# mmottl/gpr

Hardware: AMD Instinct MI355X
Metric: FITC nLML+grad training-points/sec at n=1M m=2048 d=8 (higher is better)
Workload: dtype f64

## Files before the change

### gpr_amd/csrc/gprhip.hip

```cpp
#include <algorithm>
#include <cmath>
#include <cstring>
#include <vector>
#include <string>
#include "../../include/gprhip.h"
#include "common.h"
#include "kernels.h"
#include "mfma_gemm.h"
#include "predict_plan.h"
#include "problem_internal.h"
#include "sample_paths_host.h"

static_assert(gprhip::PLAN_TILE == gprhip::TILE, "predict_plan.h rounds to the engine's tile");

namespace gprhip {
const std::string& last_error();

__global__ __launch_bounds__(256) void normalize_kernel(double* __restrict__ x, int n, double* __restrict__ nrm) {
  __shared__ double red[256];
  double s = 0.0;
  for (int i = threadIdx.x; i < n; i += 256) s += x[i] * x[i];
  red[threadIdx.x] = s;
  __syncthreads();
  for (int o = 128; o > 0; o >>= 1) {
// ... 3736 lines not shown
  }, p);
}

int gprhip_acquire_max_value(gprhip_problem* p, const double* extremes, int n_extremes, int maximise, double var_floor,
                             const double* test_inputs, int64_t ld, int64_t nt, double* values, double* dvalues, int64_t ldg,
                             double* means, double* variances, int top_k, int64_t* top_index, double* top_values,
                             double* top_dvalues, int on_device) {
  return guarded([&] {
    auto refuse = [](const char* why) {
      set_error(std::string("gprhip_acquire_max_value: ") + why);
      throw HipFail{ST_BAD_ARG};
    };
    if (n_extremes < 1 || n_extremes > GPRHIP_MAX_EXTREMES) refuse("n_extremes must lie in 1 .. GPRHIP_MAX_EXTREMES (64)");
    if (!extremes) refuse("invalid arguments (extremes is NULL)");
    for (int j = 0; j < n_extremes; ++j)
      if (!std::isfinite(extremes[j])) refuse("the extremes must be finite");
    if (!(var_floor > 0.0) || !std::isfinite(var_floor)) refuse("var_floor must be positive and finite");
    if (top_k < 0 || top_k > GPRHIP_MAX_TOP_K) refuse("top_k must lie in 0 .. GPRHIP_MAX_TOP_K (64)");
    if (top_k > 0 && !top_index) refuse("top_k > 0 needs top_index");
    if (!values && !dvalues && !means && !variances && top_k == 0)
      refuse("nothing is requested (the four outputs are NULL and top_k is 0)");
    if (!p || !test_inputs || nt < 1) refuse("invalid arguments");
    if (p->f32) refuse("the prediction gradient is evaluated in fp64 only (GPRHIP_F32_BULK problem)");
    if (p->d > 64) refuse("at most 64 point dimensions on the kernel side (d)");
    if (on_device ? ld != p->D : ld < p->D) refuse("bad ld (need ld == D for device buffers, ld >= D for host buffers)");
    if (dvalues && (on_device ? ldg != p->D : ldg < p->D))
      refuse("bad ldg (need ldg == D for device buffers, ldg >= D for host buffers)");
    do_acquire_max_value(p, extremes, n_extremes, maximise, var_floor, test_inputs, ld, nt, values, dvalues, ldg, means, variances,
                         top_k, top_index, top_values, top_dvalues, on_device);
  }, p);
}

void check_refine_options(const char* fn, const gprhip_refine_options* opt, int64_t ns, bool any_output) {
  auto refuse = [&](const std::string& why) {
    set_error(std::string(fn) + ": " + why);
    throw HipFail{ST_BAD_ARG};
  };
  if (!opt) refuse("invalid arguments (opt is NULL)");
  if (opt->max_evals < 1 || opt->max_evals > GPRHIP_REFINE_MAX_EVALS) refuse("max_evals must lie in 1 .. GPRHIP_REFINE_MAX_EVALS (1000)");
  if (!(opt->step0 > 0.0 && opt->step0 <= 1.0)) refuse("step0 must lie in (0, 1]");
  if (!(opt->c1 >= 0.0 && opt->c1 < 1.0)) refuse("c1 must lie in [0, 1)");
  if (!(opt->shrink > 0.0 && opt->shrink < 1.0)) refuse("shrink must lie in (0, 1)");
  if (!(opt->grow >= 1.0) || !std::isfinite(opt->grow)) refuse("grow must be finite and at least 1");
  if (!(opt->xtol >= 0.0) || !std::isfinite(opt->xtol)) refuse("xtol must be finite and not negative");
  if (ns < 1 || ns > GPRHIP_REFINE_MAX_STARTS) refuse("ns must lie in 1 .. GPRHIP_REFINE_MAX_STARTS (4096)");
  if (!any_output) refuse("nothing is requested (all outputs are NULL)");
}

void check_refine_box(const char* fn, const gprhip_problem* p, const double* lower, const double* upper, const double* scale,
                      int64_t ld, const double* x_out, int64_t ldx, const double* dvalues, int64_t ldg, int on_device) {
  auto refuse = [&](const std::string& why) {
    set_error(std::string(fn) + ": " + why);
    throw HipFail{ST_BAD_ARG};
  };
  const int D = p->D;
  if (on_device ? ld != D : ld < D) refuse("bad ld (need ld == D for device buffers, ld >= D for host buffers)");
  if (x_out && (on_device ? ldx != D : ldx < D)) refuse("bad ldx (need ldx == D for device buffers, ldx >= D for host buffers)");
  if (dvalues && (on_device ? ldg != D : ldg < D)) refuse("bad ldg (need ldg == D for device buffers, ldg >= D for host buffers)");
  for (int k = 0; k < D; ++k) {
    if (!std::isfinite(lower[k]) || !std::isfinite(upper[k]) || !(lower[k] < upper[k])) refuse("lower and upper must be finite with lower < upper");
    if (scale && (!(scale[k] > 0.0) || !std::isfinite(scale[k]))) refuse("scale must be positive and finite");
  }
}

std::vector<double> refine_starts(const char* fn, gprhip_problem* p, const double* starts, int64_t ld, int64_t ns, int on_device) {
  const int D = p->D;
  std::vector<double> hs((size_t)ns * D);
  if (on_device) {
    GPR_HIP(hipSetDevice(p->device));
    GPR_HIP(hipMemcpy(hs.data(), starts, hs.size() * sizeof(double), hipMemcpyDeviceToHost));
  } else {
    for (int64_t i = 0; i < ns; ++i) std::copy(starts + i * ld, starts + i * ld + D, hs.begin() + i * D);
  }
  for (double v : hs)
    if (!std::isfinite(v)) {
      set_error(std::string(fn) + ": the starts must be finite");
      throw HipFail{ST_BAD_ARG};
    }
  return hs;
}

int gprhip_acquire_refine(gprhip_problem* p, const gprhip_acquisition* acq, const gprhip_refine_options* opt, const double* lower,
                          const double* upper, const double* scale, const double* starts, int64_t ld, int64_t ns, double* x_out,
                          int64_t ldx, double* values, double* dvalues, int64_t ldg, int* evals, int* accepted, int* status,
                          double* trace, int on_device) {
  return guarded([&] {
    const char* const fn = "gprhip_acquire_refine";
    auto refuse = [&](const std::string& why) {
      set_error(std::string(fn) + ": " + why);
      throw HipFail{ST_BAD_ARG};
    };
    check_acquisition(fn, acq);
    check_refine_options(fn, opt, ns, x_out || values || dvalues || evals || accepted || status || trace);
    if (!p || !starts || !lower || !upper) refuse("invalid arguments");
    if (p->f32) refuse("the prediction gradient is evaluated in fp64 only (GPRHIP_F32_BULK problem)");
    if (p->d > 64) refuse("at most 64 point dimensions on the kernel side (d)");
    check_refine_box(fn, p, lower, upper, scale, ld, x_out, ldx, dvalues, ldg, on_device);
    need_posterior_state(p, fn, "predict from", true, acq_wants_var(acq), true,
                         "means and their gradients are available after the next gprhip_eval");
    std::vector<double> hs = refine_starts(fn, p, starts, ld, ns, on_device);
    do_acquire_refine(p, acq, opt, lower, upper, scale, starts, hs, ns, x_out, ldx, values, dvalues, ldg, evals, accepted, status,
                      trace, on_device);
  }, p);
}

int gprhip_sample_paths_refine(gprhip_problem* p, const double* z, int64_t ldz, int nd, int maximise,
                               const gprhip_refine_options* opt, const double* lower, const double* upper, const double* scale,
                               const double* starts, int64_t ld, int64_t ns, const int* draw_of, double* x_out, int64_t ldx,
                               double* values, double* dvalues, int64_t ldg, int* evals, int* accepted, int* status,
                               double* trace, int on_device) {
  return guarded([&] {
    const char* const fn = "gprhip_sample_paths_refine";
    auto refuse = [&](const std::string& why) {
      set_error(std::string(fn) + ": " + why);
      throw HipFail{ST_BAD_ARG};
    };
    if (nd < 1 || nd > GPRHIP_MAX_DRAWS) refuse("nd must lie in 1 .. GPRHIP_MAX_DRAWS (64)");
    check_refine_options(fn, opt, ns, x_out || values || dvalues || evals || accepted || status || trace);
    if (!p || !z || !starts || !draw_of || !lower || !upper) refuse("invalid arguments");
    if (p->f32) refuse("sample paths are evaluated in fp64 only (GPRHIP_F32_BULK problem)");
    if (p->d > 64) refuse("at most 64 point dimensions on the kernel side (d)");
    if (ldz < p->m) refuse("bad ldz (need ldz >= m)");
    check_refine_box(fn, p, lower, upper, scale, ld, x_out, ldx, dvalues, ldg, on_device);
    for (int64_t i = 0; i < ns; ++i)
      if (draw_of[i] < 0 || draw_of[i] >= nd) refuse("draw_of must lie in 0 .. nd - 1");
    need_posterior_state(p, fn, "draw from", true, true, true, "draws are available after the next gprhip_eval");
    std::vector<double> hs = refine_starts(fn, p, starts, ld, ns, on_device);
    do_sample_paths_refine(p, z, ldz, nd, maximise, opt, lower, upper, scale, hs, ns, draw_of, x_out, ldx, values, dvalues, ldg,
                           evals, accepted, status, trace, on_device);
  }, p);
}

int gprhip_sample_paths(gprhip_problem* p, const double* z, int64_t ldz, int ns, const double* test_inputs, int64_t ld, int64_t nt,
                        const double* eps, int64_t lde, int predictive, double* samples, int64_t lds, int maximise, int top_k,
                        int64_t* top_index, double* top_values, double* top_dvalues, int on_device) {
  return guarded([&] {
    SpCall c;
    c.have_p = p != nullptr;
    if (p) {
      c.D = p->D; c.d = p->d; c.m = p->m; c.f32 = p->f32;
    }
    c.z = z; c.ldz = ldz; c.ns = ns; c.test_inputs = test_inputs; c.ld = ld; c.nt = nt; c.eps = eps; c.lde = lde;
    c.samples = samples; c.lds = lds; c.top_k = top_k; c.top_index = top_index; c.on_device = on_device;
    if (const char* why = sp_check_args(c)) {
      set_error(std::string("gprhip_sample_paths: ") + why);
      throw HipFail{ST_BAD_ARG};
    }
    do_sample_paths(p, z, ldz, ns, test_inputs, ld, nt, eps, lde, predictive, samples, lds, maximise, top_k, top_index,
                    top_values, top_dvalues, on_device);
  }, p);
}

int gprhip_train_stats(gprhip_problem* p, double* means, double* sums) {
  return guarded([&] {
    if (!p || !sums) {
      set_error("gprhip_train_stats: invalid arguments");
      throw HipFail{ST_BAD_ARG};
    }
    if (p->f32) do_train_stats<float>(p, means, sums);
    else do_train_stats<double>(p, means, sums);
  });
}

int gprhip_covariances(gprhip_problem* p, const double* test_inputs, int64_t ld, int64_t nt, int kind,
                       int predictive, double* cov) {
  return guarded([&] {
    if (!p || !test_inputs || !cov || nt < 1 || ld < p->D || (kind != 0 && kind != 1) || nt > (1 << 20)) {
      set_error("gprhip_covariances: invalid arguments");
      throw HipFail{ST_BAD_ARG};
    }
    do_covariances(p, test_inputs, ld, nt, kind, predictive, cov);
  });
}

int gprhip_cov_samples(gprhip_problem* p, const double* cov, int64_t ld, int64_t nt, double add_diag,
                       double jitter, const double* means, const double* z, int64_t ns, double* samples) {
  return guarded([&] {
    if (!p || !cov || !means || !z || !samples || nt < 1 || ns < 1 || ld < nt || nt > (1 << 20)) {
      set_error("gprhip_cov_samples: invalid arguments");
      throw HipFail{ST_BAD_ARG};
    }
    do_cov_samples(p, cov, ld, nt, add_diag, jitter, means, z, ns, samples);
  });
}

int gprhip_co_variance_coeffs(gprhip_problem* p, double* chol_km, double* r_mat) {
  return guarded([&] {
    if (!p) {
      set_error("gprhip_co_variance_coeffs: invalid arguments");
      throw HipFail{ST_BAD_ARG};
    }
    do_co_variance_coeffs(p, chol_km, r_mat);
  });
}

int gprhip_load_predictor(gprhip_problem* p, const gprhip_hypers* h, const double* coeffs, const double* chol_km,
                          const double* r_mat) {
  return guarded([&] {
    if (!p || !h || (chol_km == nullptr) != (r_mat == nullptr) || (!coeffs && !chol_km)) {
      set_error("gprhip_load_predictor: invalid arguments");
      throw HipFail{ST_BAD_ARG};
    }
    do_load_predictor(p, h, coeffs, chol_km, r_mat);
  });
}

int gprhip_observe(gprhip_problem* p, const double* inputs, int64_t ld, const double* targets, int k, double* dlog_evidence,
                   int on_device) {
  return guarded([&] {
    const char* why = nullptr;
    if (!p || !inputs) why = "invalid arguments (problem or inputs NULL)";
    else if (k < 1 || k > GPRHIP_MAX_OBSERVE) why = "k must lie in 1 .. GPRHIP_MAX_OBSERVE (64)";
    else if (on_device ? ld != p->D : ld < p->D) why = "bad ld (need ld == D for device buffers, ld >= D for host buffers)";
    else if (p->f32) why = "the update runs in fp64 only (GPRHIP_F32_BULK problem)";
    else if (p->d > 64) why = "at most 64 point dimensions on the kernel side (d)";
    if (why) {
      set_error(std::string("gprhip_observe: ") + why);
      throw HipFail{ST_BAD_ARG};
    }
    need_observe_state(p, "gprhip_observe");
    if ((targets == nullptr) != (p->h.model_only != 0)) {
      set_error(p->h.model_only ? "gprhip_observe: the model state has no targets (model_only, or a predictor loaded without "
                                  "coefficients): targets must be NULL"
                                : "gprhip_observe: the model state has targets: targets must not be NULL");
      throw HipFail{ST_BAD_ARG};
    }
    do_observe(p, inputs, ld, targets, k, dlog_evidence, on_device);
  }, p);
}

int gprhip_posterior_save(gprhip_problem* p) {
  return guarded([&] {
    if (!p) {
      set_error("gprhip_posterior_save: NULL problem");
      throw HipFail{ST_BAD_ARG};
    }
    do_posterior_save(p);
  });
}

int gprhip_posterior_restore(gprhip_problem* p) {
  return guarded([&] {
    if (!p) {
      set_error("gprhip_posterior_restore: NULL problem");
      throw HipFail{ST_BAD_ARG};
    }
    do_posterior_restore(p);
  });
}

int64_t gprhip_observed_count(const gprhip_problem* p) { return p ? p->n_observed : 0; }

int gprhip_condition(gprhip_problem* p, double* cond_km, double* coeff_error_bound) {
  return guarded([&] {
    if (!p) {
      set_error("gprhip_condition: NULL problem");
      throw HipFail{ST_BAD_ARG};
    }
    need_model(p, "gprhip_condition");
    const double c = condition_km(p);
    if (cond_km) *cond_km = c;
    if (coeff_error_bound) *coeff_error_bound = c * (p->f32 ? 5.9604644775390625e-8 : 1.1102230246251565e-16);
  });
}

int gprhip_sync(gprhip_problem* p) {
  return guarded([&] {
    if (!p) {
      set_error("gprhip_sync: NULL problem");
      throw HipFail{ST_BAD_ARG};
    }
    GPR_HIP(hipSetDevice(p->device));
    GPR_HIP(hipStreamSynchronize(p->stream));
  });
}

void* gprhip_stream(gprhip_problem* p) { return p ? (void*)p->stream : nullptr; }

int gprhip_set_timing(gprhip_problem* p, int level) {
  return guarded([&] {
    if (!p || level < 0 || level > 2) {
      set_error("gprhip_set_timing: invalid arguments");
      throw HipFail{ST_BAD_ARG};
    }
    p->timer.kernel = level >= 1;
    p->timer.on = level >= 2;
  });
}

int gprhip_debug_fetch(gprhip_problem* p, const char* name, double* out, int64_t len) {
  return guarded([&] {
    if (!p || !out) {
      set_error("gprhip_debug_fetch: NULL argument");
      throw HipFail{ST_BAD_ARG};
    }
    const double* src = nullptr;
    int64_t avail = 0;
    std::string nm = name ? name : "";
    if (nm == "r") { src = p->r; avail = p->n; }
    else if (nm == "is") { src = p->is; avail = p->n; }
    else if (nm == "v") { src = p->v; avail = p->n; }
    else if (nm == "w") { src = p->w; avail = p->n; }
    else if (nm == "t") { src = p->tvec; avail = p->m; }
    else if (nm == "w_mat" || nm == "x_rows") {
      need_model(p, "gprhip_debug_fetch");
      if (!p->want_grad) {
        set_error("gprhip_debug_fetch: the last evaluation was evidence-only");
        throw HipFail{ST_STATE};
      }
      GPR_HIP(hipSetDevice(p->device));
      const int m = p->m, mp = p->mp;
      if (nm == "w_mat") {
        if (len < (int64_t)m * m) {
          set_error("gprhip_debug_fetch: \"w_mat\" needs m*m doubles");
          throw HipFail{ST_BAD_ARG};
        }
        std::vector<double> h((size_t)mp * mp);
        GPR_HIP(hipMemcpyAsync(h.data(), p->wmat, h.size() * sizeof(double), hipMemcpyDeviceToHost, p->stream));
        GPR_HIP(hipStreamSynchronize(p->stream));
        for (int c = 0; c < m; ++c)
          for (int r = 0; r < m; ++r) out[(size_t)c * m + r] = h[(size_t)r * mp + c];
        return;
      }
      const int64_t rows = len / m;
      if (!p->x_last || p->f32 || rows < 1 || rows > p->rows_of(0)) {
        set_error("gprhip_debug_fetch: \"x_rows\" needs an fp64 problem whose rows fit one chunk, and len = rows*m");
        throw HipFail{ST_BAD_ARG};
      }
      std::vector<double> h((size_t)rows * mp);
      GPR_HIP(hipMemcpyAsync(h.data(), p->x_last, h.size() * sizeof(double), hipMemcpyDeviceToHost, p->stream));
      GPR_HIP(hipStreamSynchronize(p->stream));
      for (int c = 0; c < m; ++c)
        for (int64_t r = 0; r < rows; ++r) out[(size_t)c * rows + r] = h[(size_t)r * mp + c];
      return;
    }
    else if (nm == "km" || nm == "knm_rows") {
      need_model(p, "gprhip_debug_fetch");
      GPR_HIP(hipSetDevice(p->device));
      const int m = p->m, mp = p->mp;
      if (nm == "km") {
        if (len < (int64_t)m * m) {
          set_error("gprhip_debug_fetch: \"km\" needs m*m doubles");
          throw HipFail{ST_BAD_ARG};
        }
        std::vector<double> h((size_t)mp * mp);
        GPR_HIP(hipMemcpyAsync(h.data(), p->km, h.size() * sizeof(double), hipMemcpyDeviceToHost, p->stream));
        GPR_HIP(hipStreamSynchronize(p->stream));
        for (int c = 0; c < m; ++c)
          for (int r = 0; r < m; ++r) out[(size_t)c * m + r] = (r <= c) ? h[(size_t)r * mp + c] : 0.0;
        return;
      }
      const int64_t rows = len / m;
      if (rows < 1 || rows > p->rows_of(0) || !p->have_inputs) {
        set_error("gprhip_debug_fetch: \"knm_rows\" needs len = rows*m with 1 <= rows <= the first row chunk");
        throw HipFail{ST_BAD_ARG};
      }
      void* const kbuf = (p->x_last == p->bufA) ? p->bufB : p->bufA;
      std::vector<double> h((size_t)rows * mp);
      if (p->f32) {
        cov_chunk<float>(p, 0, static_cast<float*>(kbuf));
        std::vector<float> hf((size_t)rows * mp);
        GPR_HIP(hipMemcpyAsync(hf.data(), kbuf, hf.size() * sizeof(float), hipMemcpyDeviceToHost, p->stream));
        GPR_HIP(hipStreamSynchronize(p->stream));
        for (size_t i = 0; i < hf.size(); ++i) h[i] = hf[i];
      } else {
        cov_chunk<double>(p, 0, static_cast<double*>(kbuf));
        GPR_HIP(hipMemcpyAsync(h.data(), kbuf, h.size() * sizeof(double), hipMemcpyDeviceToHost, p->stream));
        GPR_HIP(hipStreamSynchronize(p->stream));
      }
      for (int c = 0; c < m; ++c)
        for (int64_t r = 0; r < rows; ++r) out[(size_t)c * rows + r] = h[(size_t)r * mp + c];
      return;
    }
    else if (nm == "uinv" || nm == "rinv") {
      need_model(p, "gprhip_debug_fetch");
      if (!p->have_factors) {
        set_error("gprhip_debug_fetch: \"" + nm + "\" needs the factors of an evaluation, or of a predictor loaded with "
                  "co-variance coefficients (chol_km, r_mat)");
        throw HipFail{ST_STATE};
      }
      if (len < (int64_t)p->m * p->m) {
        set_error("gprhip_debug_fetch: \"" + nm + "\" needs m*m doubles");
        throw HipFail{ST_BAD_ARG};
      }
      GPR_HIP(hipSetDevice(p->device));
      fetch_upper_fortran(p, nm == "uinv" ? p->uinv : p->rinv, out);
      return;
    }
    else if (nm == "rtil" || nm == "bvec") {
      need_model(p, "gprhip_debug_fetch");
      if (!p->have_factors || (nm == "bvec" && (p->h.model_only || p->multi_state))) {
        set_error("gprhip_debug_fetch: \"" + nm + "\" needs the factors of an evaluation, or of a predictor loaded with "
                  "co-variance coefficients (chol_km, r_mat)" + (nm == "bvec" ? ", and a single target vector" : ""));
        throw HipFail{ST_STATE};
      }
      if (len < (nm == "rtil" ? (int64_t)p->m * p->m : (int64_t)p->m)) {
        set_error("gprhip_debug_fetch: \"" + nm + "\" needs " + (nm == "rtil" ? "m*m" : "m") + " doubles");
        throw HipFail{ST_BAD_ARG};
      }
      GPR_HIP(hipSetDevice(p->device));
      if (nm == "rtil") {
        fetch_upper_fortran(p, p->bmat, out);
        return;
      }
      if (!p->have_b) {
        DevBuf tmp;
        ensure_b(p, tmp.get<double>(p->mp));
        GPR_HIP(hipStreamSynchronize(p->stream));
      }
      GPR_HIP(hipMemcpyAsync(out, p->bvec, (size_t)p->m * sizeof(double), hipMemcpyDeviceToHost, p->stream));
      GPR_HIP(hipStreamSynchronize(p->stream));
      return;
    }
    else if (nm == "pg_m") {
      need_model(p, "gprhip_debug_fetch");
      if (!p->pg_m || !p->pg_m_valid) {
        set_error("gprhip_debug_fetch: \"pg_m\" needs M of the current model state: it is formed by the first "
                  "gprhip_predict_input_grad or gprhip_acquire call that asks for a variance part with K and G in memory");
        throw HipFail{ST_STATE};
      }
      const int64_t m = p->m, mp = p->mp;
      if (len < m * m) {
        set_error("gprhip_debug_fetch: \"pg_m\" needs m*m doubles");
        throw HipFail{ST_BAD_ARG};
      }
      const int64_t w = len >= mp * mp ? mp : m;
      GPR_HIP(hipSetDevice(p->device));
      std::vector<double> h((size_t)mp * mp);
      GPR_HIP(hipMemcpyAsync(h.data(), p->pg_m, h.size() * sizeof(double), hipMemcpyDeviceToHost, p->stream));
      GPR_HIP(hipStreamSynchronize(p->stream));
      for (int64_t c = 0; c < w; ++c)
        for (int64_t r = 0; r < w; ++r) out[(size_t)(c * w + r)] = h[(size_t)(r * mp + c)];
      return;
    }
    else if (nm == "sp_a") {
      need_model(p, "gprhip_debug_fetch");
      if (!p->sp_coef || p->sp_ns_last < 1) {
        set_error("gprhip_debug_fetch: \"sp_a\" needs the weights of a gprhip_sample_paths or gprhip_sample_paths_refine "
                  "call on the current model state");
        throw HipFail{ST_STATE};
      }
      const int64_t m = p->m, mp = p->mp, ns = p->sp_ns_last;
      if (len < m * ns) {
        set_error("gprhip_debug_fetch: \"sp_a\" needs m doubles for each draw of that call");
        throw HipFail{ST_BAD_ARG};
      }
      const bool padded = len >= mp * SP_MAX_DRAWS;
      const int64_t rows = padded ? mp : m, cols = padded ? SP_MAX_DRAWS : ns;
      GPR_HIP(hipSetDevice(p->device));
      std::vector<double> h((size_t)mp * SP_MAX_DRAWS);
      GPR_HIP(hipMemcpyAsync(h.data(), p->sp_coef + mp * SP_MAX_DRAWS, h.size() * sizeof(double), hipMemcpyDeviceToHost, p->stream));
      GPR_HIP(hipStreamSynchronize(p->stream));
      for (int64_t c = 0; c < cols; ++c)
        for (int64_t r = 0; r < rows; ++r) out[(size_t)(c * rows + r)] = h[(size_t)(r * SP_MAX_DRAWS + c)];
      return;
    }
    else {
      set_error("gprhip_debug_fetch: unknown name");
      throw HipFail{ST_BAD_ARG};
    }
    if (len > avail) len = avail;
    GPR_HIP(hipSetDevice(p->device));
    GPR_HIP(hipStreamSynchronize(p->stream));
    if (avail == p->m || p->nchunks == 1) {
      GPR_HIP(hipMemcpy(out, src, (size_t)len * sizeof(double), hipMemcpyDeviceToHost));
    } else {
      for (int c = 0; c < p->nchunks; ++c) {
        int64_t lo = (int64_t)c * p->chunk;
        if (lo >= len) break;
        int64_t cnt = std::min<int64_t>(p->rows_of(c), len - lo);
        GPR_HIP(hipMemcpy(out + lo, src + lo, (size_t)cnt * sizeof(double), hipMemcpyDeviceToHost));
      }
    }
  });
}

int gprhip_last_timings(gprhip_problem* p, const char** names, float* ms, int cap) {
  if (!p || !names || !ms) return 0;
  int n = (int)std::min<size_t>(p->tnames.size(), (size_t)cap);
  for (int i = 0; i < n; ++i) {
    names[i] = p->tnames[i].c_str();
    ms[i] = p->tms[i];
  }
  return n;
}

}
```

### gpr_amd/csrc/grad_mfma.hip

```cpp
#include "kernels.h"
#include "exp_fast.h"

namespace gprhip {

namespace {

typedef double gd4 __attribute__((ext_vector_type(4)));
__device__ __forceinline__ gd4 mfma4(double a, double b, gd4 c) {
  return __builtin_amdgcn_mfma_f64_16x16x4f64(a, b, c, 0, 0, 0);
}
__device__ __forceinline__ double wsum(double v) {
#pragma unroll
  for (int o = 32; o > 0; o >>= 1) v += __shfl_xor(v, o);
  return v;
}

constexpr int G_RC = 64;

template <int KS4, int DT, int BT, typename TS, bool KR = false>
__global__ __launch_bounds__(256, (DT + BT <= 4 && KS4 <= 8) ? 2 : 1) void grad_mfma_kernel(GradArgs<TS> a) {
  constexpr int DP = DT * 16, LDP = DP + 1;
  constexpr int BP = BT > 0 ? BT * 16 : 1, LDB = BP + 1;
  constexpr bool PF = (DT <= 2 && BT <= 2);
  constexpr int NBUF = PF ? 2 : 1;
  __shared__ double ps[KR ? 1 : NBUF * G_RC * LDP];
  __shared__ double bs[BT > 0 ? NBUF * G_RC * LDB : 1];
  __shared__ double pn[KR ? 1 : NBUF * G_RC];
  __shared__ double red[4][2];
  __shared__ double sh[DP];
  const int tid = threadIdx.x, lane = tid & 63, wv = tid >> 6;
  if (tid < DP) sh[tid] = (a.shift && tid < a.d) ? a.shift[tid] : 0.0;
  __syncthreads();
  const int l15 = lane & 15, lq = lane >> 4;
  const int cb = blockIdx.x * 128 + wv * 32;
  const ExpK ek = exp_consts();

  double zf[2][KS4], zn[2];
  bool live_c[2];
#pragma unroll
  for (int jt = 0; jt < 2; ++jt) {
    const int col = cb + jt * 16 + l15;
    live_c[jt] = col < a.m;
    double s2 = 0.0;
    if constexpr (!KR) {
#pragma unroll
      for (int s = 0; s < KS4; ++s) {
        const int k = 4 * s + lq;
        const double z = (live_c[jt] && k < a.d) ? a.Z[(int64_t)col * a.d + k] - sh[k] : 0.0;
        zf[jt][s] = z;
        s2 += z * z;
      }
      s2 += __shfl_xor(s2, 16);
      s2 += __shfl_xor(s2, 32);
    }
    zn[jt] = s2;
  }
  gd4 g[DT][2], gb[BT > 0 ? BT : 1][2];
#pragma unroll
  for (int t = 0; t < DT; ++t)
#pragma unroll
    for (int jt = 0; jt < 2; ++jt) g[t][jt] = (gd4){0, 0, 0, 0};
#pragma unroll
  for (int t = 0; t < (BT > 0 ? BT : 1); ++t)
#pragma unroll
    for (int jt = 0; jt < 2; ++jt) gb[t][jt] = (gd4){0, 0, 0, 0};
  double cs[2] = {0.0, 0.0}, sE = 0.0, sED = 0.0;

  const int r0 = blockIdx.y * a.slab;
  const int r1 = min(a.rows, r0 + a.slab);

  auto load_x = [&](int first, double (&xv)[2][4]) {
#pragma unroll
    for (int jt = 0; jt < 2; ++jt)
#pragma unroll
      for (int r = 0; r < 4; ++r) {
        const int row = first + lq + 4 * r;
        const int64_t off = (int64_t)row * a.mp + cb + jt * 16 + l15;
        if constexpr (KR) xv[jt][r] = (row < r1) ? (double)a.X[off] * (double)a.K[off] : 0.0;
        else xv[jt][r] = (row < r1) ? (double)a.X[off] : 0.0;
      }
  };
  auto tile = [&](const double* psb, const double* bsb, const double* pnb, int rb, int rt, const double (&xv)[2][4]) {
    double ev[2][4];
#pragma unroll
    for (int jt = 0; jt < 2; ++jt) {
      if constexpr (KR) {
#pragma unroll
        for (int r = 0; r < 4; ++r) {
          const double e = live_c[jt] ? xv[jt][r] : 0.0;
          ev[jt][r] = e;
          cs[jt] += e;
          sE += e;
        }
      } else {
        gd4 s4 = (gd4){0, 0, 0, 0};
#pragma unroll
        for (int s = 0; s < KS4; ++s) s4 = mfma4(psb[(rt * 16 + l15) * LDP + 4 * s + lq], zf[jt][s], s4);
#pragma unroll
        for (int r = 0; r < 4; ++r) {
          const int lr = rt * 16 + lq + 4 * r;
          const double dist = fmax(pnb[lr] + zn[jt] - 2.0 * s4[r], 0.0);
          const double kv = exp_fast(a.log_sf2 + a.inv_ell2_05 * dist, ek);
          const double e = (live_c[jt] && rb + lr < r1) ? xv[jt][r] * kv : 0.0;
          ev[jt][r] = e;
          cs[jt] += e;
          sE += e;
          sED += e * dist;
        }
      }
    }
#pragma unroll
    for (int r = 0; r < 4; ++r) {
      const int prow = (rt * 16 + 4 * r + lq);
      if (BT == 0) {
#pragma unroll
        for (int t = 0; t < DT; ++t) {
          const double ap = psb[prow * LDP + t * 16 + l15];
          g[t][0] = mfma4(ap, ev[0][r], g[t][0]);
          g[t][1] = mfma4(ap, ev[1][r], g[t][1]);
        }
      }
      if (BT > 0) {
#pragma unroll
        for (int t = 0; t < (BT > 0 ? BT : 1); ++t) {
          const double ab = bsb[prow * LDB + t * 16 + l15];
          gb[t][0] = mfma4(ab, ev[0][r], gb[t][0]);
          gb[t][1] = mfma4(ab, ev[1][r], gb[t][1]);
        }
      }
    }
  };

  if constexpr (PF) {
    constexpr int RPP = 256 / DP, NPV = G_RC / RPP;
    constexpr int RPB = 256 / BP, NBV = BT > 0 ? G_RC / RPB : 1;
    const int sr = tid / DP, sk = tid % DP;
    const int br_ = tid / BP, bk = tid % BP;
    double pv[NPV], bv[NBV];
    auto fetch_pts = [&](int rb) {
      if constexpr (!KR) {
#pragma unroll
        for (int j = 0; j < NPV; ++j) {
          const int row = rb + sr + RPP * j;
          pv[j] = (sk < a.d && row < r1) ? a.pts[(int64_t)row * a.d + sk] - sh[sk] : 0.0;
        }
      }
      if constexpr (BT > 0) {
#pragma unroll
        for (int j = 0; j < NBV; ++j) {
          const int row = rb + br_ + RPB * j;
          bv[j] = (bk < a.D && row < r1) ? a.big[(int64_t)row * a.D + bk] : 0.0;
        }
      }
    };
    auto store_pts = [&](int buf) {
      if constexpr (!KR) {
#pragma unroll
        for (int j = 0; j < NPV; ++j) {
          const int r = sr + RPP * j;
          ps[buf * G_RC * LDP + r * LDP + sk] = pv[j];
          double s2 = pv[j] * pv[j];
          s2 += __shfl_xor(s2, 1);
          s2 += __shfl_xor(s2, 2);
          s2 += __shfl_xor(s2, 4);
          s2 += __shfl_xor(s2, 8);
          if constexpr (DP == 32) s2 += __shfl_xor(s2, 16);
          if (sk == 0) pn[buf * G_RC + r] = s2;
        }
      }
      if constexpr (BT > 0) {
#pragma unroll
        for (int j = 0; j < NBV; ++j) bs[buf * G_RC * LDB + (br_ + RPB * j) * LDB + bk] = bv[j];
      }
    };
    double xv[2][4], xn[2][4];
    fetch_pts(r0);
    load_x(r0, xv);
    store_pts(0);
    __syncthreads();
    int buf = 0;
    for (int rb = r0; rb < r1; rb += G_RC, buf ^= 1) {
      const bool more = rb + G_RC < r1;
      if (more) fetch_pts(rb + G_RC);
#pragma unroll 1
      for (int rt = 0; rt < G_RC / 16; ++rt) {
        if (rb + rt * 16 >= r1) break;
        load_x(rb + rt * 16 + 16, xn);
        tile(ps + buf * G_RC * LDP, bs + (BT > 0 ? buf * G_RC * LDB : 0), pn + buf * G_RC, rb, rt, xv);
#pragma unroll
        for (int jt = 0; jt < 2; ++jt)
#pragma unroll
          for (int r = 0; r < 4; ++r) xv[jt][r] = xn[jt][r];
      }
      if (more) store_pts(buf ^ 1);
      __syncthreads();
    }
  } else {
    for (int rb = r0; rb < r1; rb += G_RC) {
      __syncthreads();
      if constexpr (!KR) {
        for (int idx = tid; idx < G_RC * DP; idx += 256) {
          const int r = idx / DP, k = idx % DP;
          ps[r * LDP + k] = (k < a.d && rb + r < r1) ? a.pts[(int64_t)(rb + r) * a.d + k] - sh[k] : 0.0;
        }
      }
      if (BT > 0) {
        for (int idx = tid; idx < G_RC * BP; idx += 256) {
          const int r = idx / BP, k = idx % BP;
          bs[r * LDB + k] = (k < a.D && rb + r < r1) ? a.big[(int64_t)(rb + r) * a.D + k] : 0.0;
        }
      }
      __syncthreads();
      if constexpr (!KR) {
        if (tid < G_RC) {
          double s2 = 0.0;
          for (int k = 0; k < DP; ++k) s2 += ps[tid * LDP + k] * ps[tid * LDP + k];
          pn[tid] = s2;
        }
        __syncthreads();
      }
#pragma unroll 1
      for (int rt = 0; rt < G_RC / 16; ++rt) {
        if (rb + rt * 16 >= r1) break;
        double xv[2][4];
        load_x(rb + rt * 16, xv);
        tile(ps, bs, pn, rb, rt, xv);
      }
    }
  }

  double* cp = a.colpart + (int64_t)blockIdx.y * a.col_rows * a.mp;
#pragma unroll
  for (int jt = 0; jt < 2; ++jt) {
    const int col = cb + jt * 16 + l15;
    double c = cs[jt];
    c += __shfl_xor(c, 16);
    c += __shfl_xor(c, 32);
    if (lq == 0) cp[col] = c;
#pragma unroll
    for (int t = 0; t < DT; ++t)
#pragma unroll
      for (int r = 0; r < 4; ++r) {
        const int dim = t * 16 + lq + 4 * r;
        if (dim < a.d) cp[(int64_t)(1 + dim) * a.mp + col] = (BT == 0) ? g[t][jt][r] + sh[dim] * c : 0.0;
      }
    if (BT > 0) {
#pragma unroll
      for (int t = 0; t < (BT > 0 ? BT : 1); ++t)
#pragma unroll
        for (int r = 0; r < 4; ++r) {
          const int dim = t * 16 + lq + 4 * r;
          if (dim < a.D) cp[(int64_t)(a.d + 1 + dim) * a.mp + col] = gb[t][jt][r];
        }
    }
  }
  sE = wsum(sE);
  sED = wsum(sED);
  if (lane == 0) {
    red[wv][0] = sE;
    red[wv][1] = sED;
  }
  __syncthreads();
  if (tid < 2)
    a.scalpart[((int64_t)blockIdx.y * gridDim.x + blockIdx.x) * 2 + tid] =
        (red[0][tid] + red[1][tid]) + (red[2][tid] + red[3][tid]);
}

template <int KS4, int DT, typename TS>
void dispatch_big(const GradArgs<TS>& a, dim3 grid, hipStream_t s) {
  if (a.K && a.big) {
    if (a.D <= 16) hipLaunchKernelGGL((grad_mfma_kernel<KS4, DT, 1, TS, true>), grid, dim3(256), 0, s, a);
    else if (a.D <= 32) hipLaunchKernelGGL((grad_mfma_kernel<KS4, DT, 2, TS, true>), grid, dim3(256), 0, s, a);
    else hipLaunchKernelGGL((grad_mfma_kernel<KS4, DT, 4, TS, true>), grid, dim3(256), 0, s, a);
    return;
  }
  if (!a.big) hipLaunchKernelGGL((grad_mfma_kernel<KS4, DT, 0, TS>), grid, dim3(256), 0, s, a);
  else if (a.D <= 16) hipLaunchKernelGGL((grad_mfma_kernel<KS4, DT, 1, TS>), grid, dim3(256), 0, s, a);
  else if (a.D <= 32) hipLaunchKernelGGL((grad_mfma_kernel<KS4, DT, 2, TS>), grid, dim3(256), 0, s, a);
  else hipLaunchKernelGGL((grad_mfma_kernel<KS4, DT, 4, TS>), grid, dim3(256), 0, s, a);
}

}

template <typename TS>
int grad_mfma_col_blocks(const GradArgs<TS>& a) {
  if (a.ms || a.d > 64 || a.D > 64 || (a.mp % 128) != 0) return 0;
  return a.mp / 128;
}

template <typename TS>
void launch_grad_mfma(const GradArgs<TS>& a, hipStream_t s) {
  dim3 grid(a.mp / 128, (a.rows + a.slab - 1) / a.slab);
  if (a.d <= 4) dispatch_big<1, 1, TS>(a, grid, s);
  else if (a.d <= 8) dispatch_big<2, 1, TS>(a, grid, s);
  else if (a.d <= 16) dispatch_big<4, 1, TS>(a, grid, s);
  else if (a.d <= 32) dispatch_big<8, 2, TS>(a, grid, s);
  else dispatch_big<16, 4, TS>(a, grid, s);
  GPR_HIP(hipGetLastError());
}

__global__ __launch_bounds__(256) void proj_inducing_grad_kernel(double* __restrict__ acc, int mp, int d, int D,
                                                                 const double* __restrict__ tproj) {
  const int c = blockIdx.x * 256 + threadIdx.x, k = blockIdx.y;
  if (c >= mp) return;
  double s = 0.0;
  for (int b = 0; b < D; ++b) s += tproj[(int64_t)k * D + b] * acc[(int64_t)(d + 1 + b) * mp + c];
  acc[(int64_t)(1 + k) * mp + c] += s;
}
void launch_proj_inducing_grad(double* acc, int mp, int d, int D, const double* tproj, hipStream_t s) {
  hipLaunchKernelGGL(proj_inducing_grad_kernel, dim3((mp + 255) / 256, d), dim3(256), 0, s, acc, mp, d, D, tproj);
  GPR_HIP(hipGetLastError());
}

template int grad_mfma_col_blocks<double>(const GradArgs<double>&);
template int grad_mfma_col_blocks<float>(const GradArgs<float>&);
template void launch_grad_mfma<double>(const GradArgs<double>&, hipStream_t);
template void launch_grad_mfma<float>(const GradArgs<float>&, hipStream_t);

}
```

Measured before the change: 2.788 million.

## Fold column sums and distance moments into the P^T E MFMA tile

For the single-tile point-dimension case (d up to 14, f64, no big features), spare columns of the shared point tile are filled with a constant one and the squared norm. The MFMA accumulation of P^T E then yields the column sum of E and the weighted norm sum alongside the gradient rows. The per-element scalar accumulations of cs, sE and sED, along with the row-bound masking in the inner loop, are removed and reconstructed once in the epilogue algebraically, with masking moved to the X load. The epilogue becomes more complex, and the rearranged summation may change floating-point rounding slightly. It also adds a debug fetch for grad_slab.

```diff
diff --git a/gpr_amd/csrc/gprhip.hip b/gpr_amd/csrc/gprhip.hip
--- a/gpr_amd/csrc/gprhip.hip
+++ b/gpr_amd/csrc/gprhip.hip
@@ -4062,6 +4062,14 @@
     else if (nm == "v") { src = p->v; avail = p->n; }
     else if (nm == "w") { src = p->w; avail = p->n; }
     else if (nm == "t") { src = p->tvec; avail = p->m; }
+    else if (nm == "grad_slab") {
+      if (len < 1) {
+        set_error("gprhip_debug_fetch: \"grad_slab\" needs one double");
+        throw HipFail{ST_BAD_ARG};
+      }
+      out[0] = (double)p->grad_slab;
+      return;
+    }
     else if (nm == "w_mat" || nm == "x_rows") {
       need_model(p, "gprhip_debug_fetch");
       if (!p->want_grad) {
diff --git a/gpr_amd/csrc/grad_mfma.hip b/gpr_amd/csrc/grad_mfma.hip
--- a/gpr_amd/csrc/grad_mfma.hip
+++ b/gpr_amd/csrc/grad_mfma.hip
@@ -1,3 +1,5 @@
+#include <type_traits>
+
 #include "kernels.h"
 #include "exp_fast.h"
 
@@ -17,8 +19,9 @@
 
 constexpr int G_RC = 64;
 
-template <int KS4, int DT, int BT, typename TS, bool KR = false>
+template <int KS4, int DT, int BT, typename TS, bool KR = false, bool MOM = false>
 __global__ __launch_bounds__(256, (DT + BT <= 4 && KS4 <= 8) ? 2 : 1) void grad_mfma_kernel(GradArgs<TS> a) {
+  static_assert(!MOM || (DT == 1 && BT == 0 && !KR), "the moment rows need two free rows in the one tile of P^T E");
   constexpr int DP = DT * 16, LDP = DP + 1;
   constexpr int BP = BT > 0 ? BT * 16 : 1, LDB = BP + 1;
   constexpr bool PF = (DT <= 2 && BT <= 2);
@@ -77,6 +80,7 @@
         const int row = first + lq + 4 * r;
         const int64_t off = (int64_t)row * a.mp + cb + jt * 16 + l15;
         if constexpr (KR) xv[jt][r] = (row < r1) ? (double)a.X[off] * (double)a.K[off] : 0.0;
+        else if constexpr (MOM) xv[jt][r] = (row < r1 && live_c[jt]) ? (double)a.X[off] : 0.0;
         else xv[jt][r] = (row < r1) ? (double)a.X[off] : 0.0;
       }
   };
@@ -101,11 +105,15 @@
           const int lr = rt * 16 + lq + 4 * r;
           const double dist = fmax(pnb[lr] + zn[jt] - 2.0 * s4[r], 0.0);
           const double kv = exp_fast(a.log_sf2 + a.inv_ell2_05 * dist, ek);
-          const double e = (live_c[jt] && rb + lr < r1) ? xv[jt][r] * kv : 0.0;
-          ev[jt][r] = e;
-          cs[jt] += e;
-          sE += e;
-          sED += e * dist;
+          if constexpr (MOM) {
+            ev[jt][r] = xv[jt][r] * kv;
+          } else {
+            const double e = (live_c[jt] && rb + lr < r1) ? xv[jt][r] * kv : 0.0;
+            ev[jt][r] = e;
+            cs[jt] += e;
+            sE += e;
+            sED += e * dist;
+          }
         }
       }
     }
@@ -143,6 +151,7 @@
         for (int j = 0; j < NPV; ++j) {
           const int row = rb + sr + RPP * j;
           pv[j] = (sk < a.d && row < r1) ? a.pts[(int64_t)row * a.d + sk] - sh[sk] : 0.0;
+          if constexpr (MOM) pv[j] = (sk == a.d && row < r1) ? 1.0 : pv[j];
         }
       }
       if constexpr (BT > 0) {
@@ -158,14 +167,15 @@
 #pragma unroll
         for (int j = 0; j < NPV; ++j) {
           const int r = sr + RPP * j;
-          ps[buf * G_RC * LDP + r * LDP + sk] = pv[j];
-          double s2 = pv[j] * pv[j];
+          if constexpr (!MOM) ps[buf * G_RC * LDP + r * LDP + sk] = pv[j];
+          double s2 = (MOM && sk >= a.d) ? 0.0 : pv[j] * pv[j];
           s2 += __shfl_xor(s2, 1);
           s2 += __shfl_xor(s2, 2);
           s2 += __shfl_xor(s2, 4);
           s2 += __shfl_xor(s2, 8);
           if constexpr (DP == 32) s2 += __shfl_xor(s2, 16);
           if (sk == 0) pn[buf * G_RC + r] = s2;
+          if constexpr (MOM) ps[buf * G_RC * LDP + r * LDP + sk] = (sk == a.d + 1) ? s2 : pv[j];
         }
       }
       if constexpr (BT > 0) {
@@ -196,6 +206,7 @@
       __syncthreads();
     }
   } else {
+    static_assert(!MOM, "one tile of point dimensions is always double-buffered");
     for (int rb = r0; rb < r1; rb += G_RC) {
       __syncthreads();
       if constexpr (!KR) {
@@ -234,8 +245,26 @@
   for (int jt = 0; jt < 2; ++jt) {
     const int col = cb + jt * 16 + l15;
     double c = cs[jt];
-    c += __shfl_xor(c, 16);
-    c += __shfl_xor(c, 32);
+    if constexpr (MOM) {
+      auto acc_row = [&](int k) {
+        const gd4 v = g[0][jt];
+        const int e = k >> 2;
+        return __shfl(e == 0 ? v[0] : e == 1 ? v[1] : e == 2 ? v[2] : v[3], (k & 3) * 16 + l15);
+      };
+      c = acc_row(a.d);
+      const double pe = acc_row(a.d + 1);
+      double dot = 0.0;
+#pragma unroll
+      for (int s = 0; s < KS4; ++s) dot += zf[jt][s] * g[0][jt][s];
+      if (lq == 0) {
+        sE += c;
+        sED += pe + zn[jt] * c;
+      }
+      sED -= 2.0 * dot;
+    } else {
+      c += __shfl_xor(c, 16);
+      c += __shfl_xor(c, 32);
+    }
     if (lq == 0) cp[col] = c;
 #pragma unroll
     for (int t = 0; t < DT; ++t)
@@ -274,7 +303,15 @@
     else hipLaunchKernelGGL((grad_mfma_kernel<KS4, DT, 4, TS, true>), grid, dim3(256), 0, s, a);
     return;
   }
-  if (!a.big) hipLaunchKernelGGL((grad_mfma_kernel<KS4, DT, 0, TS>), grid, dim3(256), 0, s, a);
+  if (!a.big) {
+    constexpr bool mom = DT == 1 && std::is_same<TS, double>::value;
+    if constexpr (mom && KS4 <= 3)
+      hipLaunchKernelGGL((grad_mfma_kernel<KS4, DT, 0, TS, false, true>), grid, dim3(256), 0, s, a);
+    else if (mom && a.d <= 14)
+      hipLaunchKernelGGL((grad_mfma_kernel<KS4, DT, 0, TS, false, mom>), grid, dim3(256), 0, s, a);
+    else
+      hipLaunchKernelGGL((grad_mfma_kernel<KS4, DT, 0, TS>), grid, dim3(256), 0, s, a);
+  }
   else if (a.D <= 16) hipLaunchKernelGGL((grad_mfma_kernel<KS4, DT, 1, TS>), grid, dim3(256), 0, s, a);
   else if (a.D <= 32) hipLaunchKernelGGL((grad_mfma_kernel<KS4, DT, 2, TS>), grid, dim3(256), 0, s, a);
   else hipLaunchKernelGGL((grad_mfma_kernel<KS4, DT, 4, TS>), grid, dim3(256), 0, s, a);
```

Result: no change. 2.787 million (-0.0%).
